# Prashant-ambati/Federated-Learning-for-Privacy-Preserving-Image-Classification

Hardware: AMD Instinct MI355X
Metric: client-images/sec/node (higher is better)
Workload: dtype f32; 1 GPU; KT: cifar10_cnn 32 clients (32/GPU), non_iid(a=0.5), 1 local epoch(s), batch 32, sgd lr 0.01, DP eps=None, FedAvg; clients=32, images_per_round=45015, batch=32, parallelism=client-packed x1 GPU

## Files before the change

federated-learning-for-privacy-preserving-image-classification_amd/csrc/bn.hip:

```cpp
#include "fh_common.h"
#include "splitbn.h"

namespace fh {

struct BNArgs {
    const float* x;
    float* y;
    const float* res;
    const float* dy;
    const float* yout;
    float* dx;
    float* dres;
    const float* gamma;
    const float* beta;
    float* rmean;
    float* rvar;
    float* save_mean;
    float* save_invstd;
    float* dgamma;
    float* dbeta;
    double* part;
    int SP;
    int64_t x_cs, y_cs, res_cs, dy_cs, yo_cs, dx_cs, dres_cs, p_cs, r_cs, g_cs;
    const int32_t* counts;
// ... 76 lines not shown
__global__ void __launch_bounds__(256) bn_apply_kernel(const BNArgs a) {
    const int s = blockIdx.x, c = blockIdx.y, z = blockIdx.z;
    const int cnt = a.counts ? a.counts[z] : a.batch;
    const int64_t n = (int64_t)cnt * a.HW;
    double sum, sq;
    merge(a, z, c, sum, sq);
    const double mean = n > 0 ? sum / (double)n : 0.0;
    double var = n > 0 ? sq / (double)n - mean * mean : 0.0;
    if (var < 0.0) var = 0.0;
    const double invstd = n > 0 ? 1.0 / sqrt(var + (double)a.eps) : 0.0;
    const float meanf = (float)mean, invstdf = (float)invstd;
    if (s == 0 && threadIdx.x == 0) {
        a.save_mean[z * a.C + c] = meanf;
        a.save_invstd[z * a.C + c] = invstdf;
        if (a.rmean && n > 0) {
            const double unb = n > 1 ? var * (double)n / (double)(n - 1) : var;
            float* rm = a.rmean + z * a.r_cs + c;
            float* rv = a.rvar + z * a.r_cs + c;
            *rm = (float)((double)a.momentum * mean + (1.0 - (double)a.momentum) * (double)*rm);
            *rv = (float)((double)a.momentum * unb + (1.0 - (double)a.momentum) * (double)*rv);
        }
    }
    const float alpha = invstdf * a.gamma[z * a.p_cs + c];
    const float bconst = a.beta[z * a.p_cs + c] - meanf * alpha;
    const float* xz = a.x + z * a.x_cs;
    float* yz = a.y + z * a.y_cs;
    const float* rz = a.res ? a.res + z * a.res_cs : nullptr;
    const int relu = a.relu;
    for_slice(a, z, c, s, [&](int64_t o, int nv) {
        if (nv == 4) {
            float4 v = ld4(xz + o);
            v.x = v.x * alpha + bconst;
            v.y = v.y * alpha + bconst;
            v.z = v.z * alpha + bconst;
            v.w = v.w * alpha + bconst;
            if (rz) {
                const float4 r = ld4(rz + o);
                v.x = v.x + r.x; v.y = v.y + r.y; v.z = v.z + r.z; v.w = v.w + r.w;
            }
            if (relu) {
                v.x = fmaxf(v.x, 0.f); v.y = fmaxf(v.y, 0.f);
                v.z = fmaxf(v.z, 0.f); v.w = fmaxf(v.w, 0.f);
            }
            st4(yz + o, v);
        } else {
            float v = xz[o] * alpha + bconst;
            if (rz) v = v + rz[o];
            if (relu) v = fmaxf(v, 0.f);
            yz[o] = v;
        }
    });
}

__global__ void __launch_bounds__(256) bn_finalize_kernel(const BNArgs a, float* scale,
                                                          float* shift, int64_t s_cs) {
    const int c = blockIdx.x * 4 + (threadIdx.x >> 6), z = blockIdx.y;
    if (c >= a.C) return;
    const int cnt = a.counts ? a.counts[z] : a.batch;
    const int64_t n = (int64_t)cnt * a.HW;
    double sum, sq;
    merge(a, z, c, sum, sq);
    if ((threadIdx.x & 63) != 0) return;
    const double mean = n > 0 ? sum / (double)n : 0.0;
    double var = n > 0 ? sq / (double)n - mean * mean : 0.0;
    if (var < 0.0) var = 0.0;
    const double invstd = n > 0 ? 1.0 / sqrt(var + (double)a.eps) : 0.0;
    const float meanf = (float)mean, invstdf = (float)invstd;
    a.save_mean[z * a.C + c] = meanf;
    a.save_invstd[z * a.C + c] = invstdf;
    if (a.rmean && n > 0) {
        const double unb = n > 1 ? var * (double)n / (double)(n - 1) : var;
        float* rm = a.rmean + z * a.r_cs + c;
        float* rv = a.rvar + z * a.r_cs + c;
        *rm = (float)((double)a.momentum * mean + (1.0 - (double)a.momentum) * (double)*rm);
        *rv = (float)((double)a.momentum * unb + (1.0 - (double)a.momentum) * (double)*rv);
    }
    const float alpha = invstdf * a.gamma[z * a.p_cs + c];
    const float bconst = a.beta[z * a.p_cs + c] - meanf * alpha;
    scale[z * s_cs + c] = alpha;
    shift[z * s_cs + c] = bconst;
}

constexpr int kPoolEpt = 4;

__global__ void __launch_bounds__(256)
maxpool2_bnfin_kernel(const BNArgs a, float* __restrict__ scale_out, float* __restrict__ shift_out,
                      int64_t s_cs, const float* __restrict__ x, int64_t x_cs,
                      float* __restrict__ y, int64_t y_cs, uint8_t* __restrict__ idx, int64_t i_cs,
                      uint8_t* __restrict__ mask, int64_t m_cs, int H, int W, int drop_mode,
                      float keep_prob, float dscale, uint64_t seed_salt,
                      const uint64_t* __restrict__ seed_dev, int bpc) {
    __shared__ float s_aff[2];
    const int z = blockIdx.y, c = blockIdx.x / bpc, sb = blockIdx.x - c * bpc;
    const int cnt = a.counts ? a.counts[z] : a.batch;
    const int64_t n = (int64_t)cnt * a.HW;
    const int OH = H / 2, OW = W / 2, ohw = OH * OW;
    const int64_t per_ch = (int64_t)cnt * ohw;
    int64_t e[kPoolEpt];
    float xv[kPoolEpt][4];
#pragma unroll
    for (int k = 0; k < kPoolEpt; ++k) {
        const int64_t q = ((int64_t)sb * kPoolEpt + k) * 256 + threadIdx.x;
        e[k] = -1;
        xv[k][0] = xv[k][1] = xv[k][2] = xv[k][3] = 0.f;
        if (q < per_ch) {
            const int img = (int)(q / ohw), r = (int)(q - (int64_t)img * ohw);
            const int oh = r / OW, ow = r - oh * OW;
            const int64_t plane = (int64_t)img * a.C + c;
            e[k] = plane * ohw + r;
            const float* pp = x + z * x_cs + plane * H * W + (2 * oh) * W + 2 * ow;
            xv[k][0] = pp[0]; xv[k][1] = pp[1]; xv[k][2] = pp[W]; xv[k][3] = pp[W + 1];
        }
    }
    if (threadIdx.x < 64) {
        const int lane = threadIdx.x;
        double s0, s1;
        merge(a, z, c, s0, s1);
        if (lane == 0) {
            const double mean = n > 0 ? s0 / (double)n : 0.0;
            double var = n > 0 ? s1 / (double)n - mean * mean : 0.0;
            if (var < 0.0) var = 0.0;
            const double invstd = n > 0 ? 1.0 / sqrt(var + (double)a.eps) : 0.0;
            const float meanf = (float)mean, invstdf = (float)invstd;
            const float alpha = invstdf * a.gamma[z * a.p_cs + c];
            const float bconst = a.beta[z * a.p_cs + c] - meanf * alpha;
            s_aff[0] = alpha;
            s_aff[1] = bconst;
            if (sb == 0) {
                a.save_mean[z * a.C + c] = meanf;
                a.save_invstd[z * a.C + c] = invstdf;
                if (a.rmean && n > 0) {
                    const double unb = n > 1 ? var * (double)n / (double)(n - 1) : var;
                    float* rm = a.rmean + z * a.r_cs + c;
                    float* rv = a.rvar + z * a.r_cs + c;
                    *rm = (float)((double)a.momentum * mean + (1.0 - (double)a.momentum) * (double)*rm);
                    *rv = (float)((double)a.momentum * unb + (1.0 - (double)a.momentum) * (double)*rv);
                }
                scale_out[z * s_cs + c] = alpha;
                shift_out[z * s_cs + c] = bconst;
            }
        }
    }
    __syncthreads();
    const float s = s_aff[0], t = s_aff[1];
    const uint64_t seed = seed_salt + (seed_dev ? *seed_dev : 0ull);
    const uint64_t prow = drop_mode == 1 ? philox_row(seed_dev, z) : 0ull;
#pragma unroll
    for (int k = 0; k < kPoolEpt; ++k) {
        if (e[k] < 0) continue;
        const float v0 = fmaxf(xv[k][0] * s + t, 0.f), v1 = fmaxf(xv[k][1] * s + t, 0.f);
        const float v2 = fmaxf(xv[k][2] * s + t, 0.f), v3 = fmaxf(xv[k][3] * s + t, 0.f);
        float m = v0;
        int am = 0;
        if (v1 > m) { m = v1; am = 1; }
        if (v2 > m) { m = v2; am = 2; }
        if (v3 > m) { m = v3; am = 3; }
        idx[z * i_cs + e[k]] = (uint8_t)am;
        if (drop_mode) {
            uint8_t keep;
            if (drop_mode == 1) {
                const uint4 rr = Philox::gen(seed, prow, (uint64_t)e[k]);
                keep = u01(rr.x) <= keep_prob ? 1 : 0;
                mask[z * m_cs + e[k]] = keep;
            } else {
                keep = mask[z * m_cs + e[k]];
            }
            m = keep ? m * dscale : 0.f;
        }
        y[z * y_cs + e[k]] = m;
    }
}

__global__ void __launch_bounds__(256) bn_eval_kernel(const BNArgs a) {
    const int s = blockIdx.x, c = blockIdx.y, z = blockIdx.z;
    const float invstd = (float)(1.0 / sqrt((double)a.rvar[z * a.r_cs + c] + (double)a.eps));
    const float alpha = invstd * a.gamma[z * a.p_cs + c];
    const float bconst = a.beta[z * a.p_cs + c] - a.rmean[z * a.r_cs + c] * alpha;
    const float* xz = a.x + z * a.x_cs;
    float* yz = a.y + z * a.y_cs;
    const float* rz = a.res ? a.res + z * a.res_cs : nullptr;
    for_slice(a, z, c, s, [&](int64_t o, int nv) {
        for (int q = 0; q < nv; ++q) {
            float v = xz[o + q] * alpha + bconst;
            if (rz) v = v + rz[o + q];
            if (a.relu) v = fmaxf(v, 0.f);
            yz[o + q] = v;
        }
    });
}


__device__ __forceinline__ float pooled_g(const BNArgs& a, int z, int64_t o) {
    uint32_t y, x;
    const int64_t plane = o / a.HW;
    a.fd_w.divmod((uint32_t)(o - plane * a.HW), y, x);
    const int64_t e = plane * (a.HW >> 2) + (int64_t)(y >> 1) * (a.W >> 1) + (x >> 1);
    if (a.pidx[z * a.pi_cs + e] != (int)(((y & 1) << 1) | (x & 1))) return 0.f;
    float g = a.dpool[z * a.dp_cs + e];
    if (a.pmask) g = a.pmask[z * a.pm_cs + e] ? g * a.pscale : 0.f;
    return g;
}

__device__ __forceinline__ float4 upstream4(const BNArgs& a, int z, int64_t o) {
    if (!a.dpool) return ld4(a.dy + z * a.dy_cs + o);
    uint32_t y, x;
    const int64_t plane = o / a.HW;
    a.fd_w.divmod((uint32_t)(o - plane * a.HW), y, x);
    const int64_t e = plane * (a.HW >> 2) + (int64_t)(y >> 1) * (a.W >> 1) + (x >> 1);
    const int r = (y & 1) << 1;
    const uint8_t* pk = a.pmask ? a.pmask + z * a.pm_cs : a.pidx + z * a.pi_cs;
    float g0 = a.dpool[z * a.dp_cs + e], g1 = a.dpool[z * a.dp_cs + e + 1];
    const int c0 = a.pidx[z * a.pi_cs + e] | (pk[e] ? 4 : 0);
    const int c1 = a.pidx[z * a.pi_cs + e + 1] | (pk[e + 1] ? 4 : 0);
    const bool dm = a.pmask != nullptr;
    const float h0 = dm ? g0 * a.pscale : g0, h1 = dm ? g1 * a.pscale : g1;
    g0 = (!dm || (c0 & 4)) ? h0 : 0.f;
    g1 = (!dm || (c1 & 4)) ? h1 : 0.f;
    const int i0 = c0 & 3, i1 = c1 & 3;
    return make_float4(i0 == r ? g0 : 0.f, i0 == (r | 1) ? g0 : 0.f, i1 == r ? g1 : 0.f,
                       i1 == (r | 1) ? g1 : 0.f);
}

__device__ __forceinline__ float upstream1(const BNArgs& a, int z, int64_t o) {
    return a.dpool ? pooled_g(a, z, o) : a.dy[z * a.dy_cs + o];
}

struct ReluMask {
    int mode;
    const float* yo;
    float alpha, bconst;
    __device__ ReluMask(const BNArgs& a, int z, int c, float mean, float invstd) {
        mode = !a.relu ? 0 : (a.yout ? 1 : 2);
        yo = mode == 1 ? a.yout + z * a.yo_cs : nullptr;
        alpha = 0.f;
        bconst = 0.f;
        if (mode == 2) {
            alpha = invstd * a.gamma[z * a.p_cs + c];
            bconst = a.beta[z * a.p_cs + c] - mean * alpha;
        }
    }
    __device__ __forceinline__ bool keep(float x, int64_t o) const {
        if (mode == 0) return true;
        if (mode == 1) return yo[o] > 0.f;
        return x * alpha + bconst > 0.f;
    }
    __device__ __forceinline__ float4 apply4(float4 g, float4 xv, int64_t o) const {
        if (mode == 0) return g;
        float4 m;
        if (mode == 1) {
            m = ld4(yo + o);
        } else {
            m.x = xv.x * alpha + bconst; m.y = xv.y * alpha + bconst;
// ... 419 lines not shown

extern "C" int fh_bn_apply_tiles(const double* part, const float* x, int64_t x_cs, float* y,
                                 int64_t y_cs, const float* res, int64_t res_cs,
                                 const float* gamma, const float* beta, int64_t p_cs,
                                 float* running_mean, float* running_var, int64_t r_cs,
                                 float* save_mean, float* save_invstd, const int32_t* counts,
                                 int32_t nclients, int32_t batch, int32_t C, int32_t HW,
                                 float eps, float momentum, int32_t relu, void* stream) {
    FH_REQUIRE(nclients >= 0 && batch > 0 && C > 0 && HW > 0, "bn_apply_tiles: bad shape");
    if (nclients == 0) return FH_OK;
    if (const int rc = sbn_settle()) return rc;
    FH_REQUIRE(part && x && y && gamma && beta && save_mean && save_invstd,
               "bn_apply_tiles: null pointer");
    FH_REQUIRE((running_mean == nullptr) == (running_var == nullptr),
               "bn_apply_tiles: running stats");
    BNArgs a = bn_args(nclients, batch, C, HW, counts);
    a.SP = (int)ceil_div((int64_t)batch * HW, 256);
    a.part = (double*)part;
    a.x = x; a.y = y; a.res = res; a.gamma = gamma; a.beta = beta;
    a.rmean = running_mean; a.rvar = running_var; a.save_mean = save_mean;
    a.save_invstd = save_invstd;
    a.x_cs = x_cs; a.y_cs = y_cs; a.res_cs = res_cs; a.p_cs = p_cs; a.r_cs = r_cs;
    a.eps = eps; a.momentum = momentum; a.relu = relu;
    FH_LAUNCH(bn_apply_kernel, dim3(a.S, C, nclients), dim3(256), 0, as_stream(stream), a);
    FH_LAUNCH_CHECK("bn_apply_tiles");
    return FH_OK;
}

extern "C" int fh_maxpool2_fwd_bnfinalize(
        const double* part, const float* gamma, const float* beta, int64_t p_cs,
        float* running_mean, float* running_var, int64_t r_cs, float* save_mean,
        float* save_invstd, float* scale_out, float* shift_out, int64_t s_cs, const float* x,
        int64_t x_cs, float* y, int64_t y_cs, uint8_t* idx, int64_t i_cs, uint8_t* mask,
        int64_t m_cs, const int32_t* counts, int32_t nclients, int32_t batch, int32_t C,
        int32_t H, int32_t W, float eps, float momentum, int32_t drop_mode, float p_drop,
        uint64_t seed, const uint64_t* seed_dev, void* stream) {
    FH_REQUIRE(nclients >= 0 && batch > 0 && C > 0 && H >= 2 && W >= 2 && !(H & 1) && !(W & 1),
               "maxpool2_fwd_bnfinalize: bad shape");
    FH_REQUIRE(drop_mode >= 0 && drop_mode <= 2 && (drop_mode == 0 || mask),
               "maxpool2_fwd_bnfinalize: mask");
    FH_REQUIRE(p_drop >= 0.f && p_drop < 1.f, "maxpool2_fwd_bnfinalize: p=%g", p_drop);
    if (nclients == 0) return FH_OK;
    FH_REQUIRE(part && gamma && beta && save_mean && save_invstd && scale_out && shift_out && x &&
               y && idx, "maxpool2_fwd_bnfinalize: null pointer");
    FH_REQUIRE((running_mean == nullptr) == (running_var == nullptr),
               "maxpool2_fwd_bnfinalize: running stats");
    BNArgs a = bn_args(nclients, batch, C, H * W, counts);
    a.S = a.SP = (int)ceil_div((int64_t)batch * H * W, 256);
    a.part = (double*)part;
    a.gamma = gamma; a.beta = beta;
    a.rmean = running_mean; a.rvar = running_var; a.save_mean = save_mean;
    a.save_invstd = save_invstd;
    a.p_cs = p_cs; a.r_cs = r_cs;
    a.eps = eps; a.momentum = momentum;
    const int64_t per_ch = (int64_t)batch * (H / 2) * (W / 2);
    const int bpc = (int)std::max<int64_t>(1, ceil_div(per_ch, 256 * kPoolEpt));
    const float keep = 1.0f - p_drop;
    SplitBnRec& r = sbn_rec();
    if (r.pending) {
        if (r.bn_part == part && r.st == as_stream(stream) && r.M == C &&
            r.sp == H * W && r.out == x && r.out_cs == x_cs && r.nclients == nclients &&
            r.batch == batch && r.counts == counts) {
            SbnFwd f{};
            f.r = r;
            f.a = a;
            f.scale = scale_out; f.shift = shift_out; f.s_cs = s_cs;
            f.ntile = a.SP;
            f.pool = 1;
            f.y = y; f.y_cs = y_cs; f.idx = idx; f.i_cs = i_cs; f.mask = mask; f.m_cs = m_cs;
            f.H = H; f.W = W; f.drop_mode = drop_mode; f.keep_prob = keep; f.dscale = 1.0f / keep;
            f.seed_salt = seed; f.seed_dev = seed_dev;
            f.fd_sp = FastDiv((uint32_t)(H * W));
            f.fd_ohw = FastDiv((uint32_t)((H / 2) * (W / 2)));
            f.fd_ow = FastDiv((uint32_t)(W / 2));
            r.pending = false;
            FH_LAUNCH(split_bnfin_kernel, dim3((unsigned)C, nclients), dim3(1024), 0,
                      as_stream(stream), f);
            FH_LAUNCH_CHECK("maxpool2_fwd_bnfinalize (split conv reduction)");
            ++g_sbn_taken;
            return FH_OK;
        }
        if (const int rc = sbn_materialize()) return rc;
    }
    FH_LAUNCH(maxpool2_bnfin_kernel, dim3((unsigned)(C * bpc), nclients), dim3(256), 0,
              as_stream(stream), a, scale_out, shift_out, s_cs, x, x_cs, y, y_cs, idx, i_cs,
              mask, m_cs, H, W, drop_mode, keep, 1.0f / keep, seed, seed_dev, bpc);
    FH_LAUNCH_CHECK("maxpool2_fwd_bnfinalize");
    return FH_OK;
}

extern "C" int fh_bn_fwd_eval(const float* x, int64_t x_cs, float* y, int64_t y_cs,
                              const float* res, int64_t res_cs, const float* gamma,
                              const float* beta, int64_t p_cs, const float* running_mean,
                              const float* running_var, int64_t r_cs, const int32_t* counts,
                              int32_t nclients, int32_t batch, int32_t C, int32_t HW, float eps,
                              int32_t relu, void* stream) {
    FH_REQUIRE(nclients >= 0 && batch > 0 && C > 0 && HW > 0, "bn_fwd_eval: bad shape");
    if (nclients == 0) return FH_OK;
    if (const int rc = sbn_settle()) return rc;
    FH_REQUIRE(x && y && gamma && beta && running_mean && running_var, "bn_fwd_eval: null pointer");
    BNArgs a = bn_args(nclients, batch, C, HW, counts);
    a.x = x; a.y = y; a.res = res; a.gamma = gamma; a.beta = beta;
    a.rmean = (float*)running_mean; a.rvar = (float*)running_var;
    a.x_cs = x_cs; a.y_cs = y_cs; a.res_cs = res_cs; a.p_cs = p_cs; a.r_cs = r_cs;
    a.eps = eps; a.relu = relu;
    FH_LAUNCH(bn_eval_kernel, dim3(a.S, C, nclients), dim3(256), 0, as_stream(stream), a);
    FH_LAUNCH_CHECK("bn_fwd_eval");
    return FH_OK;
}

extern "C" int fh_bn_bwd(const float* dy, int64_t dy_cs, const float* yout, int64_t yo_cs,
                         const float* x, int64_t x_cs, const float* gamma, const float* beta,
                         int64_t p_cs,
                         const float* save_mean, const float* save_invstd, float* dx,
                         int64_t dx_cs, float* dres, int64_t dres_cs, float* dgamma, float* dbeta,
                         int64_t g_cs, const int32_t* counts, int32_t nclients, int32_t batch,
                         int32_t C, int32_t HW, int32_t relu, void* workspace, size_t ws_bytes,
                         void* stream) {
    FH_REQUIRE(nclients >= 0 && batch > 0 && C > 0 && HW > 0, "bn_bwd: bad shape");
    if (nclients == 0) return FH_OK;
    if (const int rc = sbn_settle()) return rc;
    FH_REQUIRE(dy && x && gamma && save_mean && save_invstd, "bn_bwd: null pointer");
    FH_REQUIRE(!relu || yout || beta, "bn_bwd: relu needs the forward output or beta");
    const size_t need = fh_bn_workspace(nclients, batch, C, HW);
    FH_REQUIRE(workspace && ws_bytes >= need, "bn_bwd: workspace %zu < %zu", ws_bytes, need);
    BNArgs a = bn_args(nclients, batch, C, HW, counts);
    a.dy = dy; a.yout = yout; a.x = x; a.gamma = gamma; a.beta = beta;
    a.save_mean = (float*)save_mean;
    a.save_invstd = (float*)save_invstd; a.dx = dx; a.dres = dres; a.dgamma = dgamma;
    a.dbeta = dbeta; a.part = (double*)workspace;
    a.dy_cs = dy_cs; a.yo_cs = yo_cs; a.x_cs = x_cs; a.p_cs = p_cs; a.dx_cs = dx_cs;
    a.dres_cs = dres_cs; a.g_cs = g_cs; a.relu = relu;
    hipStream_t st = as_stream(stream);
    dim3 grid(a.S, C, nclients);
    FH_LAUNCH(bn_bwd_reduce_kernel, grid, dim3(256), 0, st, a);
    FH_LAUNCH_CHECK("bn_bwd reduce");
    FH_LAUNCH(bn_bwd_apply_kernel, grid, dim3(256), 0, st, a);
    FH_LAUNCH_CHECK("bn_bwd apply");
    return FH_OK;
}

extern "C" int fh_bn_bwd_pool(const float* dpool, int64_t dp_cs, const uint8_t* pidx,
                              int64_t pi_cs, const uint8_t* pmask, int64_t pm_cs, float p_drop,
                              const float* yout, int64_t yo_cs, const float* x, int64_t x_cs,
                              const float* gamma, const float* beta, int64_t p_cs,
                              const float* save_mean,
                              const float* save_invstd, float* dx, int64_t dx_cs, float* dgamma,
                              float* dbeta, int64_t g_cs, const int32_t* counts,
                              int32_t nclients, int32_t batch, int32_t C, int32_t H, int32_t W,
                              int32_t relu, void* workspace, size_t ws_bytes, void* stream) {
    FH_REQUIRE(nclients >= 0 && batch > 0 && C > 0 && H >= 2 && W >= 2 && !(H & 1) && !(W & 1),
               "bn_bwd_pool: bad shape");
    FH_REQUIRE(p_drop >= 0.f && p_drop < 1.f, "bn_bwd_pool: p=%g", p_drop);
    if (nclients == 0) return FH_OK;
    if (const int rc = sbn_settle()) return rc;
    FH_REQUIRE(dpool && pidx && x && gamma && save_mean && save_invstd, "bn_bwd_pool: null pointer");
    FH_REQUIRE(!relu || yout || beta, "bn_bwd_pool: relu needs the forward output or beta");
    const int HW = H * W;
    const size_t need = fh_bn_workspace(nclients, batch, C, HW);
    FH_REQUIRE(workspace && ws_bytes >= need, "bn_bwd_pool: workspace %zu < %zu", ws_bytes, need);
    BNArgs a = bn_args(nclients, batch, C, HW, counts);
    a.dpool = dpool; a.pidx = pidx; a.pmask = pmask;
    a.dp_cs = dp_cs; a.pi_cs = pi_cs; a.pm_cs = pm_cs;
    a.pscale = 1.0f / (1.0f - p_drop);
    a.W = W;
    a.fd_w = FastDiv(W);
// ... 70 lines not shown
```

federated-learning-for-privacy-preserving-image-classification_amd/csrc/layers.hip:

```cpp
#include "fh_common.h"

namespace fh {

typedef float hf32x4 __attribute__((ext_vector_type(4)));

__global__ void __launch_bounds__(256)
maxpool2_fwd_kernel(const float* __restrict__ x, int64_t x_cs, float* __restrict__ y,
                    int64_t y_cs, uint8_t* __restrict__ idx, int64_t i_cs,
                    uint8_t* __restrict__ mask, int64_t m_cs, const int32_t* __restrict__ counts,
                    int batch, int C, int H, int W, int drop_mode, float keep_prob, float scale,
                    uint64_t seed_salt, const uint64_t* __restrict__ seed_dev,
                    const float* __restrict__ in_scale, const float* __restrict__ in_shift,
                    int64_t aff_cs, int xh, int xw, int yh, int yw) {
    const uint64_t seed = seed_salt + (seed_dev ? *seed_dev : 0ull);
    const int z = blockIdx.y;
    const uint64_t prow = drop_mode == 1 ? philox_row(seed_dev, z) : 0ull;
    const int cnt = counts ? counts[z] : batch;
    const int OH = H / 2, OW = W / 2;
    const uint32_t per_img = (uint32_t)(C * OH * OW);
    const uint32_t total = (uint32_t)cnt * per_img;
    const float* xb = x + z * x_cs;
    for (uint32_t e = blockIdx.x * blockDim.x + threadIdx.x; e < total;
         e += gridDim.x * blockDim.x) {
        const uint32_t t = e / (uint32_t)OW;
// ... 723 lines not shown
}

struct NormParams {
    float mean[4];
    float stdv[4];
};

__global__ void __launch_bounds__(256)
gather_u8_kernel(const uint8_t* __restrict__ data, const int64_t* __restrict__ labels,
                 const int64_t* __restrict__ idx, int64_t idx_cs, float* __restrict__ x,
                 int64_t x_cs, int64_t* __restrict__ y, int64_t y_cs,
                 const int32_t* __restrict__ counts, int batch, int C, int H, int W,
                 NormParams np, int pad, int flip, const uchar4* __restrict__ aug_in,
                 uchar4* __restrict__ aug_out, int64_t aug_cs, uint64_t seed_salt,
                 const uint64_t* __restrict__ seed_dev) {
    const int z = blockIdx.y;
    const int cnt = counts ? counts[z] : batch;
    const uint32_t plane = (uint32_t)(H * W), per = plane * (uint32_t)C;
    const uint32_t total = (uint32_t)cnt * per;
    const uint64_t seed = seed_salt + (seed_dev ? *seed_dev : 0ull);
    const uint64_t prow = philox_row(seed_dev, z);
    constexpr int U = 4;
    const uint32_t G = gridDim.x * blockDim.x;
    const bool aug = pad > 0 || flip;
    for (uint32_t e0 = blockIdx.x * blockDim.x + threadIdx.x; e0 < total; e0 += U * G) {
        uint32_t bq[U], rq[U];
        int cq[U], sy[U], sx[U];
        int64_t sq[U];
        uchar4 aq[U];
#pragma unroll
        for (int u = 0; u < U; ++u) {
            const uint32_t e = e0 + u * G;
            const uint32_t b = e < total ? e / per : 0u;
            bq[u] = b;
            rq[u] = e - b * per;
            sq[u] = idx[z * idx_cs + b];
            aq[u] = aug_in ? aug_in[z * aug_cs + b] : make_uchar4(0, 0, 0, 0);
        }
#pragma unroll
        for (int u = 0; u < U; ++u) {
            const uint32_t e = e0 + u * G, b = bq[u], r = rq[u];
            const int c = (int)(r / plane);
            const uint32_t p = r - (uint32_t)c * plane;
            const int yy = (int)(p / (uint32_t)W), xx = (int)(p - (uint32_t)yy * (uint32_t)W);
            int ci = pad, cj = pad, fl = 0;
            if (e < total && aug) {
                if (aug_in) {
                    ci = aq[u].x; cj = aq[u].y; fl = aq[u].z;
                } else {
                    const uint4 rr = Philox::gen(seed, prow, (uint64_t)b);
                    const uint32_t span = 2u * (uint32_t)pad + 1u;
                    ci = pad > 0 ? (int)(((uint64_t)rr.x * span) >> 32) : 0;
                    cj = pad > 0 ? (int)(((uint64_t)rr.y * span) >> 32) : 0;
                    fl = flip ? (int)(rr.z >> 31) : 0;
                    if (aug_out && r == 0) aug_out[z * aug_cs + b] = make_uchar4(ci, cj, fl, 0);
                }
            }
            const int sx0 = fl ? (W - 1 - xx) : xx;
            cq[u] = c;
            sy[u] = yy + ci - pad;
            sx[u] = sx0 + cj - pad;
        }
        uint32_t ub[U];
        int64_t lq[U];
        bool inq[U];
#pragma unroll
        for (int u = 0; u < U; ++u) {
            inq[u] = e0 + u * G < total && sy[u] >= 0 && sy[u] < H && sx[u] >= 0 && sx[u] < W;
            const int64_t off = inq[u] ? ((sq[u] * H + sy[u]) * W + sx[u]) * C + cq[u] : 0;
            ub[u] = data[off];
            lq[u] = labels[sq[u]];
        }
#pragma unroll
        for (int u = 0; u < U; ++u) {
            const uint32_t e = e0 + u * G;
            if (e >= total) break;
            const float v = __fdiv_rn(inq[u] ? (float)ub[u] : 0.f, 255.f);
            x[z * x_cs + e] = __fdiv_rn(v - np.mean[cq[u]], np.stdv[cq[u]]);
            if (rq[u] == 0 && y) y[z * y_cs + bq[u]] = lq[u];
        }
    }
}

static int ew_grid(int64_t n) { return (int)std::min<int64_t>(std::max<int64_t>(ceil_div(n, 256), 1), 2048); }

}

using namespace fh;

static int maxpool2_fwd_impl(const float* x, int64_t x_cs, const float* in_scale,
                             const float* in_shift, int64_t aff_cs, float* y, int64_t y_cs,
                             uint8_t* idx, int64_t i_cs, uint8_t* mask, int64_t m_cs,
                             const int32_t* counts, int32_t nclients, int32_t batch, int32_t C,
                             int32_t H, int32_t W, int32_t drop_mode, float p_drop, uint64_t seed,
                             const uint64_t* seed_dev, void* stream, int32_t xh = 0,
                             int32_t xw = 0, int32_t yh = 0, int32_t yw = 0) {
    if (xh == 0) { xh = H; xw = W; yh = H / 2; yw = W / 2; }
    FH_REQUIRE(nclients >= 0 && batch > 0 && C > 0 && H >= 2 && W >= 2, "maxpool2_fwd: bad shape");
    FH_REQUIRE(xh >= H && xw >= W && yh >= H / 2 && yw >= W / 2, "maxpool2_fwd: plane %dx%d / "
               "%dx%d smaller than the map %dx%d", xh, xw, yh, yw, H, W);
    FH_REQUIRE((H % 2) == 0 && (W % 2) == 0, "maxpool2_fwd: odd spatial size %dx%d", H, W);
    FH_REQUIRE(drop_mode >= 0 && drop_mode <= 2 && (drop_mode == 0 || mask), "maxpool2_fwd: mask");
    FH_REQUIRE(p_drop >= 0.f && p_drop < 1.f, "maxpool2_fwd: p=%g", p_drop);
    if (nclients == 0) return FH_OK;
    FH_REQUIRE(x && y && idx, "maxpool2_fwd: null pointer");
    const float keep = 1.0f - p_drop, scale = 1.0f / keep;
    const int64_t per = (int64_t)batch * C * (H / 2) * (W / 2);
    FH_LAUNCH(maxpool2_fwd_kernel, dim3(ew_grid(per), nclients), dim3(256), 0,
                       as_stream(stream), x, x_cs, y, y_cs, idx, i_cs, mask, m_cs, counts, batch, C,
                       H, W, drop_mode, keep, scale, seed, seed_dev, in_scale, in_shift, aff_cs,
                       xh, xw, yh, yw);
    FH_LAUNCH_CHECK("maxpool2_fwd");
    return FH_OK;
}

extern "C" int fh_maxpool2_fwd(const float* x, int64_t x_cs, float* y, int64_t y_cs, uint8_t* idx,
                               int64_t i_cs, uint8_t* mask, int64_t m_cs, const int32_t* counts,
                               int32_t nclients, int32_t batch, int32_t C, int32_t H, int32_t W,
                               int32_t drop_mode, float p_drop, uint64_t seed,
                               const uint64_t* seed_dev, void* stream) {
    return maxpool2_fwd_impl(x, x_cs, nullptr, nullptr, 0, y, y_cs, idx, i_cs, mask, m_cs, counts,
                             nclients, batch, C, H, W, drop_mode, p_drop, seed, seed_dev, stream);
}

extern "C" int fh_maxpool2_fwd_bnrelu(const float* x, int64_t x_cs, const float* in_scale,
                                      const float* in_shift, int64_t aff_cs, float* y,
                                      int64_t y_cs, uint8_t* idx, int64_t i_cs, uint8_t* mask,
                                      int64_t m_cs, const int32_t* counts, int32_t nclients,
                                      int32_t batch, int32_t C, int32_t H, int32_t W,
                                      int32_t drop_mode, float p_drop, uint64_t seed,
                                      const uint64_t* seed_dev, void* stream) {
    FH_REQUIRE(in_scale && in_shift, "maxpool2_fwd_bnrelu: null scale/shift");
    return maxpool2_fwd_impl(x, x_cs, in_scale, in_shift, aff_cs, y, y_cs, idx, i_cs, mask, m_cs,
                             counts, nclients, batch, C, H, W, drop_mode, p_drop, seed, seed_dev,
                             stream);
}

static int maxpool2_bwd_impl(const float* dy, int64_t dy_cs, const uint8_t* idx, int64_t i_cs,
                             const uint8_t* mask, int64_t m_cs, float p_drop, const float* xin,
                             int64_t x_cs, float* dx, int64_t dx_cs, const int32_t* counts,
                             int32_t nclients, int32_t batch, int32_t C, int32_t H, int32_t W,
                             void* stream, int32_t gh, int32_t gw, int32_t xh, int32_t xw,
                             const float* yin = nullptr, int64_t yin_cs = 0) {
    FH_REQUIRE(nclients >= 0 && batch > 0 && C > 0 && H >= 2 && W >= 2 && !(H & 1) && !(W & 1),
               "maxpool2_bwd: bad shape");
    FH_REQUIRE(gh >= H / 2 && gw >= W / 2 && xh >= H && xw >= W, "maxpool2_bwd: plane %dx%d / "
               "%dx%d smaller than the map %dx%d", gh, gw, xh, xw, H, W);
    if (nclients == 0) return FH_OK;
    FH_REQUIRE(dy && idx && dx, "maxpool2_bwd: null pointer");
    const float scale = 1.0f / (1.0f - p_drop);
    const int64_t per = (int64_t)batch * C * (H / 2) * (W / 2);
    FH_LAUNCH(maxpool2_bwd_kernel, dim3(ew_grid(per), nclients), dim3(256), 0,
                       as_stream(stream), dy, dy_cs, idx, i_cs, mask, m_cs, xin, x_cs, dx, dx_cs,
                       counts, batch, C, H, W, scale, gh, gw, xh, xw, yin, yin_cs);
    FH_LAUNCH_CHECK("maxpool2_bwd");
    return FH_OK;
}

extern "C" int fh_maxpool2_bwd(const float* dy, int64_t dy_cs, const uint8_t* idx, int64_t i_cs,
                               const uint8_t* mask, int64_t m_cs, float p_drop, const float* xin,
                               int64_t x_cs, float* dx, int64_t dx_cs, const int32_t* counts,
                               int32_t nclients, int32_t batch, int32_t C, int32_t H, int32_t W,
                               void* stream) {
    return maxpool2_bwd_impl(dy, dy_cs, idx, i_cs, mask, m_cs, p_drop, xin, x_cs, dx, dx_cs,
                             counts, nclients, batch, C, H, W, stream, H / 2, W / 2, H, W);
}
// ... 105 lines not shown
    else
        FH_LAUNCH(linear_head_ce_kernel<false>, grid, dim3(256), 0, as_stream(stream), x, x_cs, w,
                  w_cs, bias, b_cs, targets, t_cs, logits, l_cs, dlogits, d_cs, loss_out,
                  acc_loss, acc_correct, acc_seen, reset, dw, dw_cs, db, db_cs, dx, dx_cs, mask,
                  m_cs, scale, relu_in, counts, batch, in_f, num_classes);
    FH_LAUNCH_CHECK("linear_head_ce");
    return FH_OK;
}

extern "C" int fh_eval_metrics(const float* logits, int64_t l_cs, const int64_t* targets,
                               int64_t t_cs, const int32_t* counts, int32_t nclients,
                               int32_t batch, int32_t num_classes, double* loss_sum,
                               int64_t* correct, int64_t* class_correct, int64_t* class_total,
                               void* stream) {
    FH_REQUIRE(nclients >= 0 && batch > 0 && num_classes > 0, "eval_metrics: bad shape");
    if (nclients == 0) return FH_OK;
    FH_REQUIRE(logits && targets, "eval_metrics: null pointer");
    FH_REQUIRE((class_correct == nullptr) == (class_total == nullptr),
               "eval_metrics: class_correct and class_total go together");
    FH_LAUNCH(eval_metrics_kernel, dim3(nclients), dim3(256), 0, as_stream(stream),
                       logits, l_cs, targets, t_cs, counts, batch, num_classes, loss_sum, correct,
                       reinterpret_cast<unsigned long long*>(class_correct),
                       reinterpret_cast<unsigned long long*>(class_total));
    FH_LAUNCH_CHECK("eval_metrics");
    return FH_OK;
}

extern "C" int fh_avgpool_fwd(const float* x, int64_t x_cs, float* y, int64_t y_cs,
                              const int32_t* counts, int32_t nclients, int32_t batch, int32_t C,
                              int32_t HW, void* stream) {
    FH_REQUIRE(nclients >= 0 && batch > 0 && C > 0 && HW > 0, "avgpool_fwd: bad shape");
    if (nclients == 0) return FH_OK;
    FH_REQUIRE(x && y, "avgpool_fwd: null pointer");
    const int64_t planes = (int64_t)batch * C;
    FH_LAUNCH(avgpool_fwd_kernel, dim3(ew_grid(planes * 64), nclients), dim3(256), 0,
                       as_stream(stream), x, x_cs, y, y_cs, counts, batch, C, HW);
    FH_LAUNCH_CHECK("avgpool_fwd");
    return FH_OK;
}

extern "C" int fh_avgpool_bwd(const float* dy, int64_t dy_cs, float* dx, int64_t dx_cs,
                              const int32_t* counts, int32_t nclients, int32_t batch, int32_t C,
                              int32_t HW, void* stream) {
    FH_REQUIRE(nclients >= 0 && batch > 0 && C > 0 && HW > 0, "avgpool_bwd: bad shape");
    if (nclients == 0) return FH_OK;
    FH_REQUIRE(dy && dx, "avgpool_bwd: null pointer");
    FH_LAUNCH(avgpool_bwd_kernel, dim3(ew_grid((int64_t)batch * C * HW), nclients),
                       dim3(256), 0, as_stream(stream), dy, dy_cs, dx, dx_cs, counts, batch, C, HW);
    FH_LAUNCH_CHECK("avgpool_bwd");
    return FH_OK;
}

extern "C" int fh_gather_batch(const float* data, const int64_t* labels, const int64_t* idx,
                               int64_t idx_cs, float* x, int64_t x_cs, int64_t* y, int64_t y_cs,
                               int64_t sample_elems, const int32_t* counts, int32_t nclients,
                               int32_t batch, void* stream) {
    FH_REQUIRE(nclients >= 0 && batch > 0 && sample_elems > 0, "gather_batch: bad shape");
    if (nclients == 0) return FH_OK;
    FH_REQUIRE(data && idx && x && (!y || labels), "gather_batch: null pointer");
    FH_LAUNCH(gather_kernel, dim3(ew_grid(batch * sample_elems), nclients), dim3(256), 0,
                       as_stream(stream), data, labels, idx, idx_cs, x, x_cs, y, y_cs, sample_elems,
                       counts, batch);
    FH_LAUNCH_CHECK("gather_batch");
    return FH_OK;
}

extern "C" int fh_gather_u8(const uint8_t* data, const int64_t* labels, const int64_t* idx,
                            int64_t idx_cs, float* x, int64_t x_cs, int64_t* y, int64_t y_cs,
                            const int32_t* counts, int32_t nclients, int32_t batch, int32_t C,
                            int32_t H, int32_t W, const float* mean, const float* stdv,
                            int32_t pad, int32_t flip, const uint8_t* aug_in, uint8_t* aug_out,
                            int64_t aug_cs, uint64_t seed, const uint64_t* seed_dev,
                            void* stream) {
    FH_REQUIRE(nclients >= 0 && batch > 0 && C >= 1 && C <= 4 && H > 0 && W > 0,
               "gather_u8: bad shape (C must be 1..4)");
    FH_REQUIRE(pad >= 0 && pad <= 127, "gather_u8: pad out of range");
    if (nclients == 0) return FH_OK;
    FH_REQUIRE(data && idx && x && (!y || labels) && mean && stdv, "gather_u8: null pointer");
    NormParams np;
    for (int c = 0; c < 4; ++c) {
        np.mean[c] = c < C ? mean[c] : 0.f;
        np.stdv[c] = c < C ? stdv[c] : 1.f;
    }
    FH_LAUNCH(gather_u8_kernel, dim3(ew_grid((int64_t)batch * C * H * W), nclients),
                       dim3(256), 0, as_stream(stream), data, labels, idx, idx_cs, x, x_cs, y, y_cs,
                       counts, batch, C, H, W, np, pad, flip,
                       reinterpret_cast<const uchar4*>(aug_in), reinterpret_cast<uchar4*>(aug_out),
                       aug_cs, seed, seed_dev);
    FH_LAUNCH_CHECK("gather_u8");
    return FH_OK;
}
```

Before: 292,400 client-images/s.

## Add vectorized maxpool+BN-finalize kernel and per-image LDS-staged uint8 gather

Adds a maxpool2+BN-finalize kernel for power-of-two maps with few clients. It uses float4 loads and stores, packs the argmax and dropout mask bytes into 32-bit writes, and shift-based indexing instead of divisions. It also adds a gather kernel that gives one workgroup to each image, copies the raw uint8 image into LDS with 16-byte loads, then writes normalized float4 outputs. Both aim to cut uncoalesced narrow global accesses and index arithmetic. The cost is extra code paths with alignment and shape conditions; the gather runs one block per image, and the pooling kernel handles only 4 outputs per thread.

```diff
diff --git a/federated-learning-for-privacy-preserving-image-classification_amd/csrc/bn.hip b/federated-learning-for-privacy-preserving-image-classification_amd/csrc/bn.hip
--- a/federated-learning-for-privacy-preserving-image-classification_amd/csrc/bn.hip
+++ b/federated-learning-for-privacy-preserving-image-classification_amd/csrc/bn.hip
@@ -182,6 +182,7 @@
 }
 
 constexpr int kPoolEpt = 4;
+constexpr int kPoolVecClients = 8;
 
 __global__ void __launch_bounds__(256)
 maxpool2_bnfin_kernel(const BNArgs a, float* __restrict__ scale_out, float* __restrict__ shift_out,
@@ -268,6 +269,116 @@
             m = keep ? m * dscale : 0.f;
         }
         y[z * y_cs + e[k]] = m;
+    }
+}
+
+__global__ void __launch_bounds__(256)
+maxpool2_bnfin_vec_kernel(const BNArgs a, float* __restrict__ scale_out,
+                          float* __restrict__ shift_out, int64_t s_cs, const float* __restrict__ x,
+                          int64_t x_cs, float* __restrict__ y, int64_t y_cs,
+                          uint8_t* __restrict__ idx, int64_t i_cs, uint8_t* __restrict__ mask,
+                          int64_t m_cs, int lh, int lw, int drop_mode, float keep_prob,
+                          float dscale, uint64_t seed_salt, const uint64_t* __restrict__ seed_dev,
+                          int bpc) {
+    __shared__ float s_aff[2];
+    const int z = blockIdx.y, c = blockIdx.x / bpc, sb = blockIdx.x - c * bpc;
+    const int cnt = a.counts ? a.counts[z] : a.batch;
+    const int64_t n = (int64_t)cnt * a.HW;
+    const int low = lw - 1, lohw = lh + lw - 2;
+    const int W = 1 << lw;
+    const int64_t per_ch = (int64_t)cnt << lohw;
+    constexpr int G = 1;
+    int64_t e[G];
+    float4 xa[G][2], xb[G][2];
+    uint32_t mk[G];
+#pragma unroll
+    for (int k = 0; k < G; ++k) {
+        const int64_t q = (((int64_t)sb * G + k) * 256 + threadIdx.x) * kPoolEpt;
+        e[k] = -1;
+        mk[k] = 0u;
+        xa[k][0] = xa[k][1] = xb[k][0] = xb[k][1] = make_float4(0.f, 0.f, 0.f, 0.f);
+        if (q < per_ch) {
+            const int64_t img = q >> lohw;
+            const int r = (int)(q & ((1 << lohw) - 1));
+            const int oh = r >> low, ow = r & ((1 << low) - 1);
+            const int64_t plane = img * a.C + c;
+            e[k] = (plane << lohw) + r;
+            const float* pp = x + z * x_cs + ((plane << (lh + lw)) + ((2 * oh) << lw) + 2 * ow);
+            xa[k][0] = ld4(pp); xa[k][1] = ld4(pp + 4);
+            xb[k][0] = ld4(pp + W); xb[k][1] = ld4(pp + W + 4);
+            if (drop_mode == 2) mk[k] = *reinterpret_cast<const uint32_t*>(mask + z * m_cs + e[k]);
+        }
+    }
+    if (threadIdx.x < 64) {
+        const int lane = threadIdx.x;
+        const float gam = a.gamma[z * a.p_cs + c], bet = a.beta[z * a.p_cs + c];
+        float* rm = a.rmean ? a.rmean + z * a.r_cs + c : nullptr;
+        float* rv = a.rmean ? a.rvar + z * a.r_cs + c : nullptr;
+        const float rm0 = rm ? *rm : 0.f, rv0 = rv ? *rv : 0.f;
+        double s0, s1;
+        merge(a, z, c, s0, s1);
+        if (lane == 0) {
+            const double mean = n > 0 ? s0 / (double)n : 0.0;
+            double var = n > 0 ? s1 / (double)n - mean * mean : 0.0;
+            if (var < 0.0) var = 0.0;
+            const double invstd = n > 0 ? 1.0 / sqrt(var + (double)a.eps) : 0.0;
+            const float meanf = (float)mean, invstdf = (float)invstd;
+            const float alpha = invstdf * gam;
+            const float bconst = bet - meanf * alpha;
+            s_aff[0] = alpha;
+            s_aff[1] = bconst;
+            if (sb == 0) {
+                a.save_mean[z * a.C + c] = meanf;
+                a.save_invstd[z * a.C + c] = invstdf;
+                if (rm && n > 0) {
+                    const double unb = n > 1 ? var * (double)n / (double)(n - 1) : var;
+                    *rm = (float)((double)a.momentum * mean + (1.0 - (double)a.momentum) * (double)rm0);
+                    *rv = (float)((double)a.momentum * unb + (1.0 - (double)a.momentum) * (double)rv0);
+                }
+                scale_out[z * s_cs + c] = alpha;
+                shift_out[z * s_cs + c] = bconst;
+            }
+        }
+    }
+    __syncthreads();
+    const float s = s_aff[0], t = s_aff[1];
+    const uint64_t seed = seed_salt + (seed_dev ? *seed_dev : 0ull);
+    const uint64_t prow = drop_mode == 1 ? philox_row(seed_dev, z) : 0ull;
+#pragma unroll
+    for (int k = 0; k < G; ++k) {
+        if (e[k] < 0) continue;
+        const float r0[8] = {xa[k][0].x, xa[k][0].y, xa[k][0].z, xa[k][0].w,
+                             xa[k][1].x, xa[k][1].y, xa[k][1].z, xa[k][1].w};
+        const float r1[8] = {xb[k][0].x, xb[k][0].y, xb[k][0].z, xb[k][0].w,
+                             xb[k][1].x, xb[k][1].y, xb[k][1].z, xb[k][1].w};
+        float out[kPoolEpt];
+        uint32_t ami = 0u, mko = 0u;
+#pragma unroll
+        for (int j = 0; j < kPoolEpt; ++j) {
+            const float v0 = fmaxf(r0[2 * j] * s + t, 0.f), v1 = fmaxf(r0[2 * j + 1] * s + t, 0.f);
+            const float v2 = fmaxf(r1[2 * j] * s + t, 0.f), v3 = fmaxf(r1[2 * j + 1] * s + t, 0.f);
+            float m = v0;
+            uint32_t am = 0;
+            if (v1 > m) { m = v1; am = 1; }
+            if (v2 > m) { m = v2; am = 2; }
+            if (v3 > m) { m = v3; am = 3; }
+            ami |= am << (8 * j);
+            if (drop_mode) {
+                uint32_t keep;
+                if (drop_mode == 1) {
+                    const uint4 rr = Philox::gen(seed, prow, (uint64_t)(e[k] + j));
+                    keep = u01(rr.x) <= keep_prob ? 1u : 0u;
+                    mko |= keep << (8 * j);
+                } else {
+                    keep = (mk[k] >> (8 * j)) & 0xffu;
+                }
+                m = keep ? m * dscale : 0.f;
+            }
+            out[j] = m;
+        }
+        *reinterpret_cast<uint32_t*>(idx + z * i_cs + e[k]) = ami;
+        if (drop_mode == 1) *reinterpret_cast<uint32_t*>(mask + z * m_cs + e[k]) = mko;
+        st4(y + z * y_cs + e[k], make_float4(out[0], out[1], out[2], out[3]));
     }
 }
 
@@ -853,6 +964,20 @@
         }
         if (const int rc = sbn_materialize()) return rc;
     }
+    const auto al = [](const void* p, uintptr_t m) { return (reinterpret_cast<uintptr_t>(p) & m) == 0; };
+    const auto pow2 = [](int v) { return (v & (v - 1)) == 0; };
+    if (nclients <= kPoolVecClients && pow2(H) && pow2(W) && W >= 8 && al(x, 15) && al(y, 15) && al(idx, 3) &&
+        (!mask || al(mask, 3)) && x_cs % 4 == 0 && y_cs % 4 == 0 && i_cs % 4 == 0 &&
+        (!mask || m_cs % 4 == 0)) {
+        int lh = 0, lw = 0;
+        while ((1 << lh) < H) ++lh;
+        while ((1 << lw) < W) ++lw;
+        FH_LAUNCH(maxpool2_bnfin_vec_kernel, dim3((unsigned)(C * bpc), nclients), dim3(256), 0,
+                  as_stream(stream), a, scale_out, shift_out, s_cs, x, x_cs, y, y_cs, idx, i_cs,
+                  mask, m_cs, lh, lw, drop_mode, keep, 1.0f / keep, seed, seed_dev, bpc);
+        FH_LAUNCH_CHECK("maxpool2_fwd_bnfinalize (vector)");
+        return FH_OK;
+    }
     FH_LAUNCH(maxpool2_bnfin_kernel, dim3((unsigned)(C * bpc), nclients), dim3(256), 0,
               as_stream(stream), a, scale_out, shift_out, s_cs, x, x_cs, y, y_cs, idx, i_cs,
               mask, m_cs, H, W, drop_mode, keep, 1.0f / keep, seed, seed_dev, bpc);
diff --git a/federated-learning-for-privacy-preserving-image-classification_amd/csrc/layers.hip b/federated-learning-for-privacy-preserving-image-classification_amd/csrc/layers.hip
--- a/federated-learning-for-privacy-preserving-image-classification_amd/csrc/layers.hip
+++ b/federated-learning-for-privacy-preserving-image-classification_amd/csrc/layers.hip
@@ -829,6 +829,74 @@
     }
 }
 
+constexpr int kGatherTileMax = 48 * 1024;
+
+__global__ void __launch_bounds__(256)
+gather_u8_img_kernel(const uint8_t* __restrict__ data, const int64_t* __restrict__ labels,
+                     const int64_t* __restrict__ idx, int64_t idx_cs, float* __restrict__ x,
+                     int64_t x_cs, int64_t* __restrict__ y, int64_t y_cs,
+                     const int32_t* __restrict__ counts, int batch, int C, int H, int W,
+                     NormParams np, int pad, int flip, const uchar4* __restrict__ aug_in,
+                     uchar4* __restrict__ aug_out, int64_t aug_cs, uint64_t seed_salt,
+                     const uint64_t* __restrict__ seed_dev, FastDiv fd_wq, FastDiv fd_h) {
+    extern __shared__ __align__(16) uint8_t s_img[];
+    const int z = blockIdx.y, b = blockIdx.x, tid = threadIdx.x;
+    const int cnt = counts ? counts[z] : batch;
+    if (b >= cnt) return;
+    const uint32_t plane = (uint32_t)(H * W), per = plane * (uint32_t)C;
+    const bool aug = pad > 0 || flip;
+    const int64_t sq = idx[z * idx_cs + b];
+    const uchar4 aq = aug_in ? aug_in[z * aug_cs + b] : make_uchar4(0, 0, 0, 0);
+    const uint8_t* src = data + sq * (int64_t)per;
+    if ((per & 15u) == 0) {
+        const uint4* s16 = reinterpret_cast<const uint4*>(src);
+        uint4* d16 = reinterpret_cast<uint4*>(s_img);
+        for (uint32_t w = tid; w < (per >> 4); w += 256) d16[w] = s16[w];
+    } else {
+        const uint32_t* s4 = reinterpret_cast<const uint32_t*>(src);
+        uint32_t* d4 = reinterpret_cast<uint32_t*>(s_img);
+        for (uint32_t w = tid; w < (per >> 2); w += 256) d4[w] = s4[w];
+    }
+    if (tid == 0 && y) y[z * y_cs + b] = labels[sq];
+    int ci = pad, cj = pad, fl = 0;
+    if (aug) {
+        if (aug_in) {
+            ci = aq.x; cj = aq.y; fl = aq.z;
+        } else {
+            const uint64_t seed = seed_salt + (seed_dev ? *seed_dev : 0ull);
+            const uint4 rr = Philox::gen(seed, philox_row(seed_dev, z), (uint64_t)b);
+            const uint32_t span = 2u * (uint32_t)pad + 1u;
+            ci = pad > 0 ? (int)(((uint64_t)rr.x * span) >> 32) : 0;
+            cj = pad > 0 ? (int)(((uint64_t)rr.y * span) >> 32) : 0;
+            fl = flip ? (int)(rr.z >> 31) : 0;
+            if (aug_out && tid == 0) aug_out[z * aug_cs + b] = make_uchar4(ci, cj, fl, 0);
+        }
+    }
+    __syncthreads();
+    float* xo = x + z * x_cs + (int64_t)b * per;
+    const uint32_t nq = per >> 2;
+    for (uint32_t q = tid; q < nq; q += 256) {
+        uint32_t row, xq, c, yy;
+        fd_wq.divmod(q, row, xq);
+        fd_h.divmod(row, c, yy);
+        const int sy = (int)yy + ci - pad;
+        const bool iny = sy >= 0 && sy < H;
+        const float mean = c == 0 ? np.mean[0] : c == 1 ? np.mean[1] : c == 2 ? np.mean[2] : np.mean[3];
+        const float stdv = c == 0 ? np.stdv[0] : c == 1 ? np.stdv[1] : c == 2 ? np.stdv[2] : np.stdv[3];
+        float o[4];
+#pragma unroll
+        for (int k = 0; k < 4; ++k) {
+            const int xx = (int)(xq * 4u) + k;
+            const int sx = (fl ? (W - 1 - xx) : xx) + cj - pad;
+            const bool in = iny && sx >= 0 && sx < W;
+            const uint32_t ub = s_img[in ? (uint32_t)((sy * W + sx) * C) + c : 0u];
+            const float v = __fdiv_rn(in ? (float)ub : 0.f, 255.f);
+            o[k] = __fdiv_rn(v - mean, stdv);
+        }
+        *reinterpret_cast<float4*>(xo + (int64_t)q * 4) = make_float4(o[0], o[1], o[2], o[3]);
+    }
+}
+
 static int ew_grid(int64_t n) { return (int)std::min<int64_t>(std::max<int64_t>(ceil_div(n, 256), 1), 2048); }
 
 }
@@ -1100,6 +1168,17 @@
         np.mean[c] = c < C ? mean[c] : 0.f;
         np.stdv[c] = c < C ? stdv[c] : 1.f;
     }
+    const int64_t per = (int64_t)C * H * W;
+    const auto al16 = [](const void* p) { return (reinterpret_cast<uintptr_t>(p) & 15u) == 0; };
+    if (al16(data) && al16(x) && x_cs % 4 == 0 && W % 4 == 0 && per <= kGatherTileMax) {
+        FH_LAUNCH(gather_u8_img_kernel, dim3((unsigned)batch, nclients), dim3(256),
+                  (size_t)((per + 15) & ~(int64_t)15), as_stream(stream), data, labels, idx, idx_cs,
+                  x, x_cs, y, y_cs, counts, batch, C, H, W, np, pad, flip,
+                  reinterpret_cast<const uchar4*>(aug_in), reinterpret_cast<uchar4*>(aug_out),
+                  aug_cs, seed, seed_dev, FastDiv((uint32_t)(W / 4)), FastDiv((uint32_t)H));
+        FH_LAUNCH_CHECK("gather_u8 (image per workgroup)");
+        return FH_OK;
+    }
     FH_LAUNCH(gather_u8_kernel, dim3(ew_grid((int64_t)batch * C * H * W), nclients),
                        dim3(256), 0, as_stream(stream), data, labels, idx, idx_cs, x, x_cs, y, y_cs,
                        counts, batch, C, H, W, np, pad, flip,
```

New measurement: 295,000 client-images/s, median of 6. About the same (+0.9%).
